# AdrianoEttari/DiffusionRemoteSensing

Measured on AMD Instinct MI355X. Metric: unet_denoise_steps_per_s, higher is better.
Workload: dtype f16 main + block-scaled fp6 (e2m3) cross terms of tap pairs on the wide 3x3 layers (FL, 11 of 11 launches of the dominant kernel); split bf16 x3 (hi + lo) everywhere else; f32 accumulate

## Files before the change

diffusionremotesensing_amd/csrc/attn_gate_sp.hip:

```cpp
#include "conv_epilogue.h"
#include "mfma_policy.h"

namespace {

template <int NT, bool PSI_ONLY = false>
__global__ __launch_bounds__(NT == 2 ? 1024 : 512, 1) void attn_gate_sp_kernel(AttnGateDesc d) {
  constexpr int THREADS = NT == 2 ? 1024 : 512, NW = THREADS / 64;
  extern __shared__ __attribute__((aligned(16))) char smem[];
  using P = PolicyBF16X3;
  constexpr int Ch = 16 * NT, NC = NT / 2;
  const int ncx = d.Cc / 32;
  const int gate_img = ncx * 4 * Ch * 16, wg_img = NC * 4 * Ch * 16, wx_img = NC * 16 * Ch * 16;
  char* sGate = smem;
  char* sWg = sGate + 2 * gate_img;
  char* sWx = sWg + 2 * wg_img;
  char* sRes = sWx + 2 * wx_img;
  float* sB = reinterpret_cast<float*>(sRes + 2 * wg_img);
  {
    const int tid = threadIdx.x;
    auto copy = [&](char* dst, const void* src, int bytes) {
      for (int o0 = tid * 16; o0 < bytes; o0 += 8 * THREADS * 16) {
        u32x4 v[8];
#pragma unroll
        for (int u = 0; u < 8; ++u) {
          const int o = o0 + u * THREADS * 16;
          if (o < bytes) v[u] = *reinterpret_cast<const u32x4*>(reinterpret_cast<const char*>(src) + o);
        }
#pragma unroll
        for (int u = 0; u < 8; ++u) {
          const int o = o0 + u * THREADS * 16;
          if (o < bytes) *reinterpret_cast<u32x4*>(dst + o) = v[u];
        }
      }
    };
    copy(sGate, d.w_gate, 2 * gate_img);
    copy(sWg, d.w_wg, 2 * wg_img);
    copy(sWx, d.w_wx, 2 * wx_img);
    if constexpr (!PSI_ONLY) copy(sRes, d.w_res, 2 * wg_img);
    for (int i = tid; i < Ch; i += THREADS) {
      sB[i] = d.b_gate[i];
      sB[Ch + i] = d.b_wg[i] + d.b_wx[i];
      sB[2 * Ch + i] = d.w_psi[i];
      sB[3 * Ch + i] = PSI_ONLY ? 0.f : d.b_res[i];
    }
    if (tid == 0) sB[4 * Ch] = d.b_psi[0];
  }
  __syncthreads();

  const int lane = threadIdx.x & 63, wave = threadIdx.x >> 6;
  const int lr = lane & 15, kg = lane >> 4;
  auto wfrag = [&](const char* base, int img, int slot) {
    return P::load(base, (size_t)img, (size_t)slot * 16);
  };
  const int bw = (d.LW + 15) / 16;
  const long long nitems = (long long)d.N * d.LH * bw;
  const int OW = 2 * d.LW, OH = 2 * d.LH;
  for (long long it = (long long)blockIdx.x * NW + wave; it < nitems; it += (long long)gridDim.x * NW) {
    const int xb = (int)(it % bw), y = (int)((it / bw) % d.LH), n = (int)(it / ((long long)bw * d.LH));
    const int px_raw = xb * 16 + lr;
    const bool valid = px_raw < d.LW;
    const int px = valid ? px_raw : d.LW - 1;
    typename P::Frag xr[4][NC];
#pragma unroll
    for (int t = 0; t < 4; ++t) {
      const size_t pix = ((size_t)n * OH + 2 * y + (t >> 1)) * OW + 2 * px + (t & 1);
      const char* g = reinterpret_cast<const char*>(d.xres) + (pix * d.r_cs + d.r_co) * 4 + kg * 16;
#pragma unroll
      for (int cc = 0; cc < NC; ++cc)
        xr[t][cc] = typename P::Frag{*reinterpret_cast<const bf16x8*>(g + cc * 128), *reinterpret_cast<const bf16x8*>(g + cc * 128 + 64)};
    }
    f32x4 acc[NT];
#pragma unroll
    for (int tt = 0; tt < NT; ++tt) acc[tt] = f32x4{0.f, 0.f, 0.f, 0.f};
    {
      const char* g = reinterpret_cast<const char*>(d.x) + ((((size_t)n * d.LH + y) * d.LW + px) * d.x_cs + d.x_co) * 4 + kg * 16;
      for (int c = 0; c < ncx; c += 2) {
        const typename P::Frag a0{*reinterpret_cast<const bf16x8*>(g + c * 128), *reinterpret_cast<const bf16x8*>(g + c * 128 + 64)};
        const typename P::Frag a1{*reinterpret_cast<const bf16x8*>(g + c * 128 + 128), *reinterpret_cast<const bf16x8*>(g + c * 128 + 192)};
#pragma unroll
        for (int tt = 0; tt < NT; ++tt) acc[tt] = P::mma(wfrag(sGate, gate_img, (c * 4 + kg) * Ch + tt * 16 + lr), a0, acc[tt]);
#pragma unroll
        for (int tt = 0; tt < NT; ++tt) acc[tt] = P::mma(wfrag(sGate, gate_img, ((c + 1) * 4 + kg) * Ch + tt * 16 + lr), a1, acc[tt]);
      }
    }
    typename P::Frag gfr[NC];
#pragma unroll
    for (int cc = 0; cc < NC; ++cc) {
      const float* bsrc = d.b_gate_img ? d.b_gate_img + (size_t)n * Ch + cc * 32 + kg * 8 : sB + cc * 32 + kg * 8;
      const float4 b0 = *reinterpret_cast<const float4*>(bsrc);
      const float4 b1 = *reinterpret_cast<const float4*>(bsrc + 4);
      const float bb[8] = {b0.x, b0.y, b0.z, b0.w, b1.x, b1.y, b1.z, b1.w};
      float v[8];
#pragma unroll
      for (int j = 0; j < 4; ++j) {
        v[j] = drs_maxf(acc[2 * cc][j] + bb[j], 0.f);
        v[4 + j] = drs_maxf(acc[2 * cc + 1][j] + bb[4 + j], 0.f);
      }
      u32x4 h, l;
      drs_sp_split8(v, h, l);
      gfr[cc] = typename P::Frag{__builtin_bit_cast(bf16x8, h), __builtin_bit_cast(bf16x8, l)};
    }
#pragma unroll
    for (int tt = 0; tt < NT; ++tt) acc[tt] = f32x4{0.f, 0.f, 0.f, 0.f};
#pragma unroll
    for (int cc = 0; cc < NC; ++cc)
#pragma unroll
      for (int tt = 0; tt < NT; ++tt) acc[tt] = P::mma(wfrag(sWg, wg_img, (cc * 4 + kg) * Ch + tt * 16 + lr), gfr[cc], acc[tt]);
    __builtin_amdgcn_sched_barrier(0);
#pragma unroll
    for (int t = 0; t < 4; ++t) {
#pragma unroll
      for (int cc = 0; cc < NC; ++cc)
#pragma unroll
        for (int tt = 0; tt < NT; ++tt)
          acc[tt] = P::mma(wfrag(sWx, wx_img, ((cc * 4 + t) * 4 + kg) * Ch + tt * 16 + lr), xr[t][cc], acc[tt]);
      __builtin_amdgcn_sched_barrier(0);
    }
    float dot = 0.f;
#pragma unroll
    for (int tt = 0; tt < NT; ++tt) {
      const int ch = (tt >> 1) * 32 + kg * 8 + (tt & 1) * 4;
      const float4 bs = *reinterpret_cast<const float4*>(sB + Ch + ch);
      const float4 wp = *reinterpret_cast<const float4*>(sB + 2 * Ch + ch);
      dot += drs_maxf(acc[tt][0] + bs.x, 0.f) * wp.x + drs_maxf(acc[tt][1] + bs.y, 0.f) * wp.y +
             drs_maxf(acc[tt][2] + bs.z, 0.f) * wp.z + drs_maxf(acc[tt][3] + bs.w, 0.f) * wp.w;
    }
    dot += __shfl_xor(dot, 16);
    dot += __shfl_xor(dot, 32);
    const float psi = 1.f / (1.f + expf(-(dot + sB[4 * Ch])));
    if (d.psi_out && valid && kg == 0) d.psi_out[((size_t)n * d.LH + y) * d.LW + px] = psi;
    if constexpr (!PSI_ONLY)
#pragma unroll
    for (int t = 0; t < 4; ++t) {
#pragma unroll
      for (int tt = 0; tt < NT; ++tt) acc[tt] = f32x4{0.f, 0.f, 0.f, 0.f};
#pragma unroll
      for (int cc = 0; cc < NC; ++cc)
#pragma unroll
        for (int tt = 0; tt < NT; ++tt) acc[tt] = P::mma(wfrag(sRes, wg_img, (cc * 4 + kg) * Ch + tt * 16 + lr), xr[t][cc], acc[tt]);
      __builtin_amdgcn_sched_barrier(0);
      const size_t pix = ((size_t)n * OH + 2 * y + (t >> 1)) * OW + 2 * px + (t & 1);
      char* o = reinterpret_cast<char*>(d.out) + (pix * d.out_cs + d.out_co) * 4 + kg * 16;
#pragma unroll
      for (int cc = 0; cc < NC; ++cc) {
        const float4 b0 = *reinterpret_cast<const float4*>(sB + 3 * Ch + cc * 32 + kg * 8);
        const float4 b1 = *reinterpret_cast<const float4*>(sB + 3 * Ch + cc * 32 + kg * 8 + 4);
        const float bb[8] = {b0.x, b0.y, b0.z, b0.w, b1.x, b1.y, b1.z, b1.w};
        float v[8];
#pragma unroll
        for (int j = 0; j < 4; ++j) {
          v[j] = psi * acc[2 * cc][j] + bb[j];
          v[4 + j] = psi * acc[2 * cc + 1][j] + bb[4 + j];
        }
        u32x4 h, l;
        drs_sp_split8(v, h, l);
        if (valid) {
          drs_store16(o + cc * 128, h);
          drs_store16(o + cc * 128 + 64, l);
        }
      }
    }
  }
}


template <int NCX>
__global__ __launch_bounds__(512, 1) void attn_gate_wide2_kernel(AttnGateDesc d) {
  using P = PolicyBF16X3;
  using Frag = typename P::Frag;
  constexpr int Ch = 128, NG = 4;
  constexpr int XB = 4 * NCX * 16 * 128;
  constexpr int TB = 4 * NG * 16 * 128;
  constexpr int RB = XB > 2 * TB ? XB : 2 * TB;
  extern __shared__ __attribute__((aligned(16))) char smem[];
  char* sX = smem;
  char* sG = smem + RB;
  float* sPsi = reinterpret_cast<float*>(sG + TB);
  float* sB = sPsi + 8 * 64;
  for (int i = threadIdx.x; i < Ch; i += 512) {
    sB[i] = d.b_wg[i] + d.b_wx[i];
    sB[Ch + i] = d.w_psi[i];
    sB[2 * Ch + i] = d.b_res[i];
  }
  if (threadIdx.x == 0) sB[3 * Ch] = d.b_psi[0];
  const int tid = threadIdx.x, lane = tid & 63, wave = __builtin_amdgcn_readfirstlane((int)(tid >> 6));
  const int lr = lane & 15, kg = lane >> 4;
  const int G = wave >> 1, th = wave & 1, ch0 = G * 32 + kg * 8 + th * 4;
  const size_t gate_img = (size_t)NCX * 4 * Ch * 16, wg_img = (size_t)NG * 4 * Ch * 16, wx_img = (size_t)NG * 16 * Ch * 16;
  const int bw = (d.LW + 15) / 16;
  const long long nblk16 = (long long)d.N * d.LH * bw;
  const long long nitems = (nblk16 + 3) / 4;
  const int OW = 2 * d.LW, OH = 2 * d.LH;
  typedef const __attribute__((address_space(1))) char* gptr;
  typedef const __attribute__((address_space(1))) bf16x8* gfrag;
  typedef const __attribute__((address_space(1))) u32x4* gquad;
  auto uni = [](const void* q) __attribute__((always_inline)) {
    gptr g = (gptr)q;
    asm volatile("" : "+s"(g));
    return g;
  };
  const gptr gw_gate = uni(d.w_gate), gw_wg = uni(d.w_wg), gw_wx = uni(d.w_wx), gw_res = uni(d.w_res);
  const gptr gx = uni(reinterpret_cast<const char*>(d.x) + (size_t)d.x_co * 4);
  const gptr gr = uni(reinterpret_cast<const char*>(d.xres) + (size_t)d.r_co * 4);
  const unsigned lane_w = (unsigned)((kg * Ch + wave * 16 + lr) * 16);
  auto opaque = [](unsigned v) __attribute__((always_inline)) { asm volatile("" : "+v"(v)); return v; };
  auto wfrag = [&](gptr base, size_t img, int urow) __attribute__((always_inline)) {
    const unsigned o = opaque(lane_w) + (unsigned)urow * (unsigned)(Ch * 16);
    return Frag{*(gfrag)(base + o), *(gfrag)(base + (o + (unsigned)img))};
  };
  auto afrag = [&](const char* img, int nc, int pb, int c) __attribute__((always_inline)) {
    const char* line = img + ((pb * nc + c) * 16 + lr) * 128;
    const int s0 = ((kg + lr) & 7) * 16;
    return Frag{*reinterpret_cast<const bf16x8*>(line + s0), *reinterpret_cast<const bf16x8*>(line + (s0 ^ 64))};
  };
  auto mfma = [](const bf16x8& w, const bf16x8& x, const f32x4& c) __attribute__((always_inline)) {
    return __builtin_amdgcn_mfma_f32_16x16x32_bf16(w, x, c, 0, 0, 0);
  };
  auto step4 = [&](const Frag& w, const Frag (&a)[4], f32x4 (&acc)[4]) __attribute__((always_inline)) {
#pragma unroll
    for (int b = 0; b < 4; ++b) acc[b] = mfma(w.lo, a[b].hi, acc[b]);
#pragma unroll
    for (int b = 0; b < 4; ++b) acc[b] = mfma(w.hi, a[b].lo, acc[b]);
#pragma unroll
    for (int b = 0; b < 4; ++b) acc[b] = mfma(w.hi, a[b].hi, acc[b]);
  };
  __syncthreads();
  for (long long it = blockIdx.x; it < nitems; it += gridDim.x) {
    unsigned xo[4], ro[4], oo[4];
    int nn[4], npx[4];
#pragma unroll
    for (int b = 0; b < 4; ++b) {
      const long long q = it * 4 + b;
      const long long qc = q < nblk16 ? q : nblk16 - 1;
      const int xb = (int)(qc % bw), y = (int)((qc / bw) % d.LH);
      nn[b] = (int)(qc / ((long long)bw * d.LH));
      npx[b] = q < nblk16 ? min(16, d.LW - xb * 16) : 0;
      xo[b] = (unsigned)((((size_t)nn[b] * d.LH + y) * d.LW + xb * 16) * d.x_cs * 4);
      ro[b] = (unsigned)((((size_t)nn[b] * OH + 2 * y) * OW + 2 * xb * 16) * d.r_cs * 4);
      oo[b] = (unsigned)((((size_t)nn[b] * OH + 2 * y) * OW + 2 * xb * 16) * d.out_cs * 4);
    }
    auto pick = [&](const unsigned (&v)[4], int b) __attribute__((always_inline)) { return b == 0 ? v[0] : b == 1 ? v[1] : b == 2 ? v[2] : v[3]; };
    auto picki = [&](const int (&v)[4], int b) __attribute__((always_inline)) { return b == 0 ? v[0] : b == 1 ? v[1] : b == 2 ? v[2] : v[3]; };
    u32x4 xr[8];
#pragma unroll
    for (int i = 0; i < 8; ++i) {
      const int e = i * 512 + tid, pix = e / (8 * NCX), pb = pix >> 4, pl = pix & 15;
      const int plc = min(pl, max(picki(npx, pb) - 1, 0));
      xr[i] = *(gquad)(gx + (pick(xo, pb) + (unsigned)(plc * d.x_cs * 4) + (unsigned)((e % (8 * NCX)) * 16)));
    }
    u32x4 tr[4];
    auto tap_load = [&](int t4) __attribute__((always_inline)) {
#pragma unroll
      for (int i = 0; i < 4; ++i) {
        const int e = i * 512 + tid, pix = e >> 5, pb = pix >> 4, pl = pix & 15;
        const int plc = min(pl, max(picki(npx, pb) - 1, 0));
        tr[i] = *(gquad)(gr + (pick(ro, pb) + (unsigned)((((t4 >> 1) * OW + 2 * plc + (t4 & 1)) * d.r_cs) * 4) + (unsigned)((e & 31) * 16)));
      }
    };
    auto tap_store = [&](int buf) __attribute__((always_inline)) {
#pragma unroll
      for (int i = 0; i < 4; ++i) {
        const int e = i * 512 + tid, pix = e >> 5, c = (e >> 3) & 3, sl = e & 7, pb = pix >> 4, pl = pix & 15;
        *reinterpret_cast<u32x4*>(sX + buf * TB + ((pb * NG + c) * 16 + pl) * 128 + ((sl + pl) & 7) * 16) = tr[i];
      }
    };
    tap_load(0);
    Frag wr[NG];
#pragma unroll
    for (int cc = 0; cc < NG; ++cc) wr[cc] = wfrag(gw_res, wg_img, cc * 4);
    constexpr int WD = 3, NST = NCX + NG + 4 * NG;
    Frag wq[WD + 1];
    auto wstep = [&](int st) __attribute__((always_inline)) {
      if (st < NCX) return wfrag(gw_gate, gate_img, st * 4);
      if (st < NCX + NG) return wfrag(gw_wg, wg_img, (st - NCX) * 4);
      const int t4 = (st - NCX - NG) / NG, cc = (st - NCX - NG) % NG;
      return wfrag(gw_wx, wx_img, (cc * 4 + t4) * 4);
    };
#pragma unroll
    for (int st = 0; st < WD; ++st) wq[st] = wstep(st);
#pragma unroll
    for (int i = 0; i < 8; ++i) {
      const int e = i * 512 + tid, pix = e / (8 * NCX), c = (e / 8) % NCX, sl = e & 7, pb = pix >> 4, pl = pix & 15;
      *reinterpret_cast<u32x4*>(sX + ((pb * NCX + c) * 16 + pl) * 128 + ((sl + pl) & 7) * 16) = xr[i];
    }
    __syncthreads();
    f32x4 acc[4];
#pragma unroll
    for (int b = 0; b < 4; ++b) acc[b] = f32x4{0.f, 0.f, 0.f, 0.f};
#pragma unroll
    for (int c = 0; c < NCX; ++c) {
      if (c + WD < NST) wq[(c + WD) % (WD + 1)] = wstep(c + WD);
      Frag a[4];
#pragma unroll
      for (int b = 0; b < 4; ++b) a[b] = afrag(sX, NCX, b, c);
      step4(wq[c % (WD + 1)], a, acc);
      __builtin_amdgcn_sched_barrier(0);
    }
    {
#pragma unroll
      for (int b = 0; b < 4; ++b) {
        const float* bsrc = (d.b_gate_img ? d.b_gate_img + (size_t)nn[b] * Ch : d.b_gate) + ch0;
        const float4 bb = *reinterpret_cast<const float4*>(bsrc);
        const float v[4] = {drs_maxf(acc[b][0] + bb.x, 0.f), drs_maxf(acc[b][1] + bb.y, 0.f), drs_maxf(acc[b][2] + bb.z, 0.f), drs_maxf(acc[b][3] + bb.w, 0.f)};
        unsigned h2[2], l2[2];
        drs_sp_split4(v, h2, l2);
        char* line = sG + ((b * NG + G) * 16 + lr) * 128;
        const int s0 = ((kg + lr) & 7) * 16 + th * 8;
        *reinterpret_cast<uint2*>(line + s0) = make_uint2(h2[0], h2[1]);
        *reinterpret_cast<uint2*>(line + (s0 ^ 64)) = make_uint2(l2[0], l2[1]);
      }
    }
    __syncthreads();
    tap_store(0);
    tap_load(1);
    __syncthreads();
#pragma unroll
    for (int b = 0; b < 4; ++b) acc[b] = f32x4{0.f, 0.f, 0.f, 0.f};
#pragma unroll
    for (int cc = 0; cc < NG; ++cc) {
      if (NCX + cc + WD < NST) wq[(NCX + cc + WD) % (WD + 1)] = wstep(NCX + cc + WD);
      Frag a[4];
#pragma unroll
      for (int b = 0; b < 4; ++b) a[b] = afrag(sG, NG, b, cc);
      step4(wq[(NCX + cc) % (WD + 1)], a, acc);
      __builtin_amdgcn_sched_barrier(0);
    }
    f32x4 att[4][4];
#pragma unroll
    for (int t4 = 0; t4 < 4; ++t4)
#pragma unroll
      for (int b = 0; b < 4; ++b) att[t4][b] = f32x4{0.f, 0.f, 0.f, 0.f};
#pragma unroll
    for (int t4 = 0; t4 < 4; ++t4) {
      if (t4 + 1 < 4) tap_store((t4 + 1) & 1);
      if (t4 + 2 < 4) tap_load(t4 + 2);
#pragma unroll
      for (int cc = 0; cc < NG; ++cc) {
        const int st = NCX + NG + t4 * NG + cc;
        if (st + WD < NST) wq[(st + WD) % (WD + 1)] = wstep(st + WD);
        Frag a[4];
#pragma unroll
        for (int b = 0; b < 4; ++b) a[b] = afrag(sX + (t4 & 1) * TB, NG, b, cc);
        step4(wq[st % (WD + 1)], a, acc);
        step4(wr[cc], a, att[t4]);
        __builtin_amdgcn_sched_barrier(0);
      }
      __syncthreads();
    }
    {
      const float4 bsum = *reinterpret_cast<const float4*>(sB + ch0), wp = *reinterpret_cast<const float4*>(sB + Ch + ch0);
#pragma unroll
      for (int b = 0; b < 4; ++b) {
        float dot = drs_maxf(acc[b][0] + bsum.x, 0.f) * wp.x + drs_maxf(acc[b][1] + bsum.y, 0.f) * wp.y +
                    drs_maxf(acc[b][2] + bsum.z, 0.f) * wp.z + drs_maxf(acc[b][3] + bsum.w, 0.f) * wp.w;
        dot += __shfl_xor(dot, 16);
        dot += __shfl_xor(dot, 32);
        if (kg == 0) sPsi[wave * 64 + b * 16 + lr] = dot;
      }
    }
    __syncthreads();
    {
      const float4 br = *reinterpret_cast<const float4*>(sB + 2 * Ch + ch0);
#pragma unroll
      for (int b = 0; b < 4; ++b) {
        const int i = b * 16 + lr;
        float sum = sB[3 * Ch];
#pragma unroll
        for (int w = 0; w < 8; ++w) sum += sPsi[w * 64 + i];
        const float psi = 1.f / (1.f + expf(-sum));
        const bool ok = lr < npx[b];
        if (d.psi_out && ok && kg == 0 && wave == 0) {
          const long long q = it * 4 + b;
          const int xb = (int)(q % bw), y = (int)((q / bw) % d.LH);
          d.psi_out[((size_t)nn[b] * d.LH + y) * d.LW + xb * 16 + lr] = psi;
        }
#pragma unroll
        for (int t4 = 0; t4 < 4; ++t4) {
          const float v[4] = {psi * att[t4][b][0] + br.x, psi * att[t4][b][1] + br.y, psi * att[t4][b][2] + br.z, psi * att[t4][b][3] + br.w};
          unsigned h2[2], l2[2];
          drs_sp_split4(v, h2, l2);
          if (ok) {
            char* o = reinterpret_cast<char*>(d.out) + (size_t)d.out_co * 4 + oo[b] +
                      (size_t)(((t4 >> 1) * OW + 2 * lr + (t4 & 1)) * d.out_cs + G * 32) * 4 + kg * 16 + th * 8;
            *reinterpret_cast<uint2*>(o) = make_uint2(h2[0], h2[1]);
            *reinterpret_cast<uint2*>(o + 64) = make_uint2(l2[0], l2[1]);
// ... 97 lines not shown
```

diffusionremotesensing_amd/csrc/conv_s2_sp.hip:

```cpp
#include <stdio.h>
#include <stdlib.h>

#include "conv_epilogue.h"
#include "mfma_policy.h"

namespace {

__device__ __forceinline__ void copy_weights(char* smem, const TapConv& d, int nck, int GC, int n0, unsigned w_gimage, int tid) {
  const int slots = nck * 36 * GC;
  const char* wsrc = reinterpret_cast<const char*>(d.w);
  for (int i0 = tid; i0 < 2 * slots; i0 += 512 * 8) {
    u32x4 v[8];
#pragma unroll
    for (int u = 0; u < 8; ++u) {
      const int i = i0 + u * 512;
      if (i < 2 * slots) {
        const int im = i >= slots, idx = im ? i - slots : i;
        const int r = idx / GC, j = idx - r * GC;
        v[u] = *reinterpret_cast<const u32x4*>(wsrc + (size_t)im * w_gimage + ((size_t)r * d.Cout + n0 + j) * 16);
      }
    }
#pragma unroll
    for (int u = 0; u < 8; ++u) {
      const int i = i0 + u * 512;
      if (i < 2 * slots) *reinterpret_cast<u32x4*>(smem + (size_t)i * 16) = v[u];
    }
  }
}

template <int NT>
__global__ __launch_bounds__(512, 1) void conv_s2_sp_kernel(TapConv d, int nck, unsigned w_gimage) {
  extern __shared__ __attribute__((aligned(16))) char smem[];
  using P = PolicyBF16X3;
  constexpr int GC = 16 * NT;
  const int tid = threadIdx.x, lane = tid & 63, wave = __builtin_amdgcn_readfirstlane(tid >> 6);
  const int lr = lane & 15, kg = lane >> 4;
  const int ngroups = d.Cout / GC;
  const int xcd = blockIdx.x & 7, j8 = blockIdx.x >> 3, nb8 = gridDim.x >> 3;
  const int grp = j8 % ngroups, member = j8 / ngroups, members = nb8 / ngroups;
  const int n0 = grp * GC;
  const int img = nck * 36 * GC * 16;
  copy_weights(smem, d, nck, GC, n0, w_gimage, tid);
  __syncthreads();

  const int bw = (d.OW + 15) / 16;
  const int rows = d.N * d.OH;
  const int r_lo = (int)((long long)rows * xcd / 8), r_hi = (int)((long long)rows * (xcd + 1) / 8);
  const int Q = (r_hi - r_lo) * bw;
  const int stride = members * 8, first = member * 8 + wave;
  const int my_items = first < Q ? (Q - first + stride - 1) / stride : 0;
  const int S = my_items * nck;
  if (S == 0) return;
  const int half = drs_sp_group_bytes(d.in_cs);
  const char* zero = reinterpret_cast<const char*>(d.zero_line) + kg * 16;
  const char* wbase = smem + ((size_t)kg * GC + lr) * 16;

  struct Taps { typename P::Frag c[3], r[3], e[3]; };
  Taps fa, fb;
  auto issue = [&](int s, Taps& f) __attribute__((always_inline)) {
    const int it = s / nck, c = s - it * nck;
    const int q = first + it * stride;
    const int row = r_lo + q / bw, xb = q - (q / bw) * bw;
    const int n = row / d.OH, y = row - n * d.OH;
    const int px = min(xb * 16 + lr, d.OW - 1);
    const int iy0 = 2 * y - 1, ix0 = 2 * px - 1;
    const char* base = reinterpret_cast<const char*>(d.in) +
                       ((((long long)n * d.H + iy0) * d.W + ix0) * d.in_cs + d.in_co) * 4 + c * 128 + kg * 16;
    const int rowb = d.W * d.in_cs * 4, pixb = d.in_cs * 4;
#pragma unroll
    for (int ky = 0; ky < 3; ++ky) {
      const bool row_ok = ky > 0 || iy0 >= 0;
      const char* pc = row_ok ? base + ky * rowb + pixb : zero;
      const char* pr = row_ok ? base + ky * rowb + 2 * pixb : zero;
      f.c[ky] = typename P::Frag{*reinterpret_cast<const bf16x8*>(pc), *reinterpret_cast<const bf16x8*>(row_ok ? pc + half : zero)};
      f.r[ky] = typename P::Frag{*reinterpret_cast<const bf16x8*>(pr), *reinterpret_cast<const bf16x8*>(row_ok ? pr + half : zero)};
      if (lr == 0) {
        const bool ok = row_ok && ix0 >= 0;
        const char* pe = ok ? base + ky * rowb : zero;
        f.e[ky] = typename P::Frag{*reinterpret_cast<const bf16x8*>(pe), *reinterpret_cast<const bf16x8*>(ok ? pe + half : zero)};
      }
    }
  };
  auto shift_in = [&](const bf16x8& edge, const bf16x8& right) __attribute__((always_inline)) {
    const u32x4 e = __builtin_bit_cast(u32x4, edge), r = __builtin_bit_cast(u32x4, right);
    u32x4 o;
#pragma unroll
    for (int j = 0; j < 4; ++j)
      o[j] = (unsigned)__builtin_amdgcn_update_dpp((int)e[j], (int)r[j], 0x111, 0xf, 0xf, false);
    return __builtin_bit_cast(bf16x8, o);
  };
  f32x4 acc[1][NT];
  float bias8[NT / 2][8];
#pragma unroll
  for (int pr = 0; pr < NT / 2; ++pr) {
    const float4 a = d.bias ? *reinterpret_cast<const float4*>(d.bias + n0 + pr * 32 + kg * 8) : make_float4(0.f, 0.f, 0.f, 0.f);
    const float4 b = d.bias ? *reinterpret_cast<const float4*>(d.bias + n0 + pr * 32 + kg * 8 + 4) : make_float4(0.f, 0.f, 0.f, 0.f);
    bias8[pr][0] = a.x; bias8[pr][1] = a.y; bias8[pr][2] = a.z; bias8[pr][3] = a.w;
    bias8[pr][4] = b.x; bias8[pr][5] = b.y; bias8[pr][6] = b.z; bias8[pr][7] = b.w;
  }
  auto store_row = [&](int n, int y, int x0) __attribute__((always_inline)) {
    const bool lo = lr < 8;
    const int pl = lr & 7;
#pragma unroll
    for (int pr = 0; pr < NT / 2; ++pr) {
      float v[8];
#pragma unroll
      for (int j = 0; j < 4; ++j) { v[j] = acc[0][2 * pr][j] + bias8[pr][j]; v[4 + j] = acc[0][2 * pr + 1][j] + bias8[pr][4 + j]; }
      if (d.relu_pre || d.relu_post) {
#pragma unroll
        for (int j = 0; j < 8; ++j) v[j] = drs_maxf(v[j], 0.f);
      }
      u32x4 H, L;
      drs_sp_split8(v, H, L);
      const u32x4 got = drs_dpp_swap8(lo ? L : H);
#pragma unroll
      for (int h = 0; h < 2; ++h) {
        const int tx = x0 + pl + 8 * h;
        if (tx < d.OW) {
          const size_t opix = ((size_t)n * d.OH + y) * d.OW + tx;
          char* gp = reinterpret_cast<char*>(d.out) + (opix * d.out_cs + d.out_co + n0 + pr * 32) * 4 + (lo ? 0 : 64) + kg * 16;
          drs_store16(gp, (h == 0) ? (lo ? H : got) : (lo ? got : L));
        }
      }
    }
  };
  auto compute = [&](int s, const Taps& f) __attribute__((always_inline)) {
    const int it = s / nck, c = s - it * nck;
    if (c == 0) {
#pragma unroll
      for (int t = 0; t < NT; ++t) acc[0][t] = f32x4{0.f, 0.f, 0.f, 0.f};
    }
    const char* wc = wbase + (size_t)c * 36 * GC * 16;
#pragma unroll
    for (int ky = 0; ky < 3; ++ky) {
      const typename P::Frag left{shift_in(f.e[ky].hi, f.r[ky].hi), shift_in(f.e[ky].lo, f.r[ky].lo)};
#pragma unroll
      for (int kx = 0; kx < 3; ++kx) {
        const typename P::Frag& a = kx == 0 ? left : (kx == 1 ? f.c[ky] : f.r[ky]);
#pragma unroll
        for (int t = 0; t < NT; ++t) {
          const typename P::Frag wf = P::load(wc, (size_t)img, (size_t)((ky * 3 + kx) * 4 * GC + t * 16) * 16);
          acc[0][t] = P::mma(wf, a, acc[0][t]);
        }
      }
      __builtin_amdgcn_sched_barrier(0);
    }
    if (c == nck - 1) {
      const int q = first + it * stride;
      const int row = r_lo + q / bw, xb = q - (q / bw) * bw;
      const int n = row / d.OH, y = row - n * d.OH;
      store_row(n, y, xb * 16);
    }
  };
  issue(0, fa);
  for (int s = 0; s < S; s += 2) {
    if (s + 1 < S) issue(s + 1, fb);
    compute(s, fa);
    if (s + 2 < S) issue(s + 2, fa);
    if (s + 1 < S) compute(s + 1, fb);
  }
}


template <int NT>
__global__ __launch_bounds__(512, 1) void convt_sp_kernel(TapConv d, int nck, unsigned w_gimage) {
  extern __shared__ __attribute__((aligned(16))) char smem[];
  using P = PolicyBF16X3;
  constexpr int GC = 16 * NT;
  const int tid = threadIdx.x, lane = tid & 63, wave = __builtin_amdgcn_readfirstlane(tid >> 6);
  const int lr = lane & 15, kg = lane >> 4;
  const int ngroups = d.Cout / GC;
  const int xcd = blockIdx.x & 7, j8 = blockIdx.x >> 3, nb8 = gridDim.x >> 3;
  const int grp = j8 % ngroups, member = j8 / ngroups, members = nb8 / ngroups;
  const int n0 = grp * GC;
  const int img = nck * 36 * GC * 16;
  copy_weights(smem, d, nck, GC, n0, w_gimage, tid);
  __syncthreads();

  const int bw = d.W / 16;
  const int rows = d.N * (d.H >> 1);
  const int r_lo = (int)((long long)rows * xcd / 8), r_hi = (int)((long long)rows * (xcd + 1) / 8);
  const int Q = (r_hi - r_lo) * bw;
  const int stride = members * 8, first = member * 8 + wave;
  const int my_items = first < Q ? (Q - first + stride - 1) / stride : 0;
  const int S = my_items * nck;
  if (S == 0) return;
  const int half = drs_sp_group_bytes(d.in_cs);
  const char* zero = reinterpret_cast<const char*>(d.zero_line) + kg * 16;
  const char* wbase = smem + ((size_t)kg * GC + lr) * 16;

  struct Rows { typename P::Frag a[3], e[3]; };
  Rows fa, fb;
  auto issue = [&](int s, Rows& f) __attribute__((always_inline)) {
    const int it = s / nck, c = s - it * nck;
    const int q = first + it * stride;
    const int row = r_lo + q / bw, xb = q - (q / bw) * bw;
    const int hh = d.H >> 1;
    const int n = row / hh, y = 2 * (row - n * hh);
    const int px = xb * 16 + lr;
    const char* base = reinterpret_cast<const char*>(d.in) +
                       ((((long long)n * d.H + y) * d.W + px) * d.in_cs + d.in_co) * 4 + c * 128 + kg * 16;
    const int rowb = d.W * d.in_cs * 4, pixb = d.in_cs * 4;
#pragma unroll
    for (int dy = 0; dy < 3; ++dy) {
      const bool row_ok = y + dy < d.H;
      const char* p = row_ok ? base + dy * rowb : zero;
      f.a[dy] = typename P::Frag{*reinterpret_cast<const bf16x8*>(p), *reinterpret_cast<const bf16x8*>(row_ok ? p + half : zero)};
      if (lr == 15) {
        const bool ok = row_ok && px + 1 < d.W;
        const char* pe = ok ? base + dy * rowb + pixb : zero;
        f.e[dy] = typename P::Frag{*reinterpret_cast<const bf16x8*>(pe), *reinterpret_cast<const bf16x8*>(ok ? pe + half : zero)};
      }
    }
  };
  auto shift_in = [&](const bf16x8& edge, const bf16x8& own) __attribute__((always_inline)) {
    const u32x4 e = __builtin_bit_cast(u32x4, edge), r = __builtin_bit_cast(u32x4, own);
    u32x4 o;
#pragma unroll
    for (int j = 0; j < 4; ++j)
      o[j] = (unsigned)__builtin_amdgcn_update_dpp((int)e[j], (int)r[j], 0x101, 0xf, 0xf, false);
    return __builtin_bit_cast(bf16x8, o);
  };
  f32x4 acc[2][4][NT];
  float bias8[NT / 2][8];
#pragma unroll
  for (int pr = 0; pr < NT / 2; ++pr) {
    const float4 a = d.bias ? *reinterpret_cast<const float4*>(d.bias + n0 + pr * 32 + kg * 8) : make_float4(0.f, 0.f, 0.f, 0.f);
    const float4 b = d.bias ? *reinterpret_cast<const float4*>(d.bias + n0 + pr * 32 + kg * 8 + 4) : make_float4(0.f, 0.f, 0.f, 0.f);
    bias8[pr][0] = a.x; bias8[pr][1] = a.y; bias8[pr][2] = a.z; bias8[pr][3] = a.w;
    bias8[pr][4] = b.x; bias8[pr][5] = b.y; bias8[pr][6] = b.z; bias8[pr][7] = b.w;
  }
  auto store_item = [&](int r, int n, int y, int x0) __attribute__((always_inline)) {
    const bool lo = lr < 8;
    const int pl = lr & 7;
#pragma unroll
    for (int ph = 0; ph < 4; ++ph)
#pragma unroll
      for (int pr = 0; pr < NT / 2; ++pr) {
        float v[8];
#pragma unroll
        for (int j = 0; j < 4; ++j) { v[j] = acc[r][ph][2 * pr][j] + bias8[pr][j]; v[4 + j] = acc[r][ph][2 * pr + 1][j] + bias8[pr][4 + j]; }
        u32x4 H, L;
        drs_sp_split8(v, H, L);
        const u32x4 got = drs_dpp_swap8(lo ? L : H);
        const size_t orow = ((size_t)n * d.OH + 2 * y + (ph >> 1)) * d.OW;
#pragma unroll
        for (int h = 0; h < 2; ++h) {
          const size_t opix = orow + 2 * (x0 + pl + 8 * h) + (ph & 1);
          char* gp = reinterpret_cast<char*>(d.out) + (opix * d.out_cs + d.out_co + n0 + pr * 32) * 4 + (lo ? 0 : 64) + kg * 16;
          drs_store16(gp, (h == 0) ? (lo ? H : got) : (lo ? got : L));
        }
      }
  };
  auto compute = [&](int s, const Rows& f) __attribute__((always_inline)) {
    const int it = s / nck, c = s - it * nck;
    if (c == 0) {
#pragma unroll
      for (int r = 0; r < 2; ++r)
#pragma unroll
        for (int ph = 0; ph < 4; ++ph)
#pragma unroll
          for (int t = 0; t < NT; ++t) acc[r][ph][t] = f32x4{0.f, 0.f, 0.f, 0.f};
    }
    const char* wc = wbase + (size_t)c * 36 * GC * 16;
    typename P::Frag right[3];
#pragma unroll
    for (int i = 0; i < 3; ++i) right[i] = typename P::Frag{shift_in(f.e[i].hi, f.a[i].hi), shift_in(f.e[i].lo, f.a[i].lo)};
#pragma unroll
    for (int dy = 0; dy < 2; ++dy) {
#pragma unroll
      for (int dx = 0; dx < 2; ++dx) {
#pragma unroll
        for (int ky = 0; ky < 3; ++ky)
#pragma unroll
          for (int kx = 0; kx < 3; ++kx) {
            if ((ky == 0 ? 1 : 0) != dy || (kx == 0 ? 1 : 0) != dx) continue;
            const int ph = (ky == 1 ? 0 : 1) * 2 + (kx == 1 ? 0 : 1);
#pragma unroll
            for (int t = 0; t < NT; ++t) {
              const typename P::Frag wf = P::load(wc, (size_t)img, (size_t)((ky * 3 + kx) * 4 * GC + t * 16) * 16);
#pragma unroll
              for (int r = 0; r < 2; ++r) acc[r][ph][t] = P::mma(wf, dx == 0 ? f.a[r + dy] : right[r + dy], acc[r][ph][t]);
            }
          }
        __builtin_amdgcn_sched_barrier(0);
      }
    }
    if (c == nck - 1) {
      const int q = first + it * stride;
      const int row = r_lo + q / bw, xb = q - (q / bw) * bw;
      const int hh = d.H >> 1;
      const int n = row / hh, y = 2 * (row - n * hh);
      store_item(0, n, y, xb * 16);
      store_item(1, n, y + 1, xb * 16);
    }
  };
  issue(0, fa);
  for (int s = 0; s < S; s += 2) {
    if (s + 1 < S) issue(s + 1, fb);
    compute(s, fa);
    if (s + 2 < S) issue(s + 2, fa);
    if (s + 1 < S) compute(s + 1, fb);
  }
}

template <int NT, bool CONVT = false>
int s2_launch(const TapConv& d, int nck, unsigned w_gimage, hipStream_t s) {
  auto kern = CONVT ? convt_sp_kernel<2> : conv_s2_sp_kernel<NT>;
  const size_t lds = (size_t)2 * nck * 36 * 16 * NT * 16;
  int num_cu = 0;
  {
    const int rc = drs_kernel_prepare(reinterpret_cast<const void*>(kern), 160 * 1024, &num_cu);
    if (rc) return rc;
  }
  const int ngroups = d.Cout / (16 * NT);
  int per_xcd = num_cu / 8;
  per_xcd = per_xcd / ngroups * ngroups;
  if (per_xcd < ngroups) per_xcd = ngroups;
  DRS_LAUNCH(kern, dim3((unsigned)(8 * per_xcd)), dim3(512), lds, s, d, nck, w_gimage);
  DRS_CHECK_HIP(hipGetLastError());
  return DRS_OK;
}

int s2_tiles(const TapConv& d) {
  const int nck = d.Cin / 32;
  const size_t budget = 156 * 1024;
  if (d.Cout % 64 == 0 && d.Cout <= 64 && (size_t)2 * nck * 36 * 64 * 16 <= budget) return 4;
  if ((size_t)2 * nck * 36 * 32 * 16 <= budget) return 2;
  return 0;
}

}

bool drs_conv_s2_sp_supported(const TapConv& d, int impl) {
  static const int env = getenv("DRS_S2K") ? atoi(getenv("DRS_S2K")) : 1;
  if (!env || impl != DRS_IMPL_MFMA_BF16X3) return false;
  if (!d.in || !d.in_sp || !d.out || !d.out_sp || !d.zero_line || d.mode != 0 || d.ntaps != 9 || d.wtaps_total != 9) return false;
  if (d.in_stride != 2 || d.out_scale != 1 || d.out_oy || d.out_ox) return false;
  for (int i = 0; i < 9; ++i)
    if (d.dy[i] != i / 3 - 1 || d.dx[i] != i % 3 - 1 || d.wtap[i] != i) return false;
  if (d.in2 || d.out2 || d.fuse_out || d.dual || d.gate || d.in_add || d.res || d.sigmoid || d.out_nchw) return false;
  if ((d.H & 1) || (d.W & 1) || d.OH != d.H / 2 || d.OW != d.W / 2 || d.TH != d.OH || d.TW != d.OW) return false;
  if (d.Cin % 32 || d.Cout % 32 || (d.in_cs & 31) || (d.in_co & 31) || (d.out_cs & 31) || (d.out_co & 31)) return false;
  if (d.post_add || d.bias2) return false;
  return s2_tiles(d) != 0;
}

int drs_launch_conv_s2_sp(const TapConv& d, hipStream_t s) {
  const int nck = d.Cin / 32;
  const unsigned w_gimage = (unsigned)((size_t)nck * 9 * 4 * d.Cout * 16);
  return s2_tiles(d) == 4 ? s2_launch<4>(d, nck, w_gimage, s) : s2_launch<2>(d, nck, w_gimage, s);
}

bool drs_convt_sp_supported(const TapConv& d, int impl) {
  static const int env = getenv("DRS_S2K") ? atoi(getenv("DRS_S2K")) : 1;
  if (!env || impl != DRS_IMPL_MFMA_BF16X3) return false;
  if (!d.in || !d.in_sp || !d.out || !d.out_sp || !d.zero_line || d.mode != DRS_TAPMODE_CONVT || d.ntaps != 9 || d.wtaps_total != 9) return false;
  if (d.in_stride != 1 || d.out_scale != 2 || d.out_oy || d.out_ox) return false;
  for (int i = 0; i < 9; ++i)
    if (d.wtap[i] != i) return false;
  if (d.in2 || d.out2 || d.fuse_out || d.dual || d.gate || d.in_add || d.res || d.sigmoid || d.out_nchw) return false;
  if (d.post_add || d.bias2 || d.relu_pre || d.relu_post) return false;
  if ((d.W & 15) || (d.H & 1) || d.OH != 2 * d.H || d.OW != 2 * d.W || d.TH != d.H || d.TW != d.W) return false;
  if (d.Cin % 32 || d.Cout % 32 || (d.in_cs & 31) || (d.in_co & 31) || (d.out_cs & 31) || (d.out_co & 31)) return false;
  return (size_t)2 * (d.Cin / 32) * 36 * 32 * 16 <= 156 * 1024;
}

int drs_launch_convt_sp(const TapConv& d, hipStream_t s) {
  const int nck = d.Cin / 32;
  const unsigned w_gimage = (unsigned)((size_t)nck * 9 * 4 * d.Cout * 16);
  return s2_launch<2, true>(d, nck, w_gimage, s);
}
```

diffusionremotesensing_amd/csrc/upfuse_proj_sp.hip:

```cpp
#include <stdio.h>
#include <stdlib.h>

#include "conv_epilogue.h"
#include "mfma_policy.h"

namespace {

constexpr int RBC = 8;
struct RowOpU { PolicyBF16X3::Frag c, e; };

__device__ __forceinline__ bf16x8 dpp_shift_u(const bf16x8& edge, const bf16x8& own, bool left) {
  const u32x4 e = __builtin_bit_cast(u32x4, edge), r = __builtin_bit_cast(u32x4, own);
  u32x4 o;
#pragma unroll
  for (int j = 0; j < 4; ++j)
    o[j] = left ? (unsigned)__builtin_amdgcn_update_dpp((int)e[j], (int)r[j], 0x111, 0xf, 0xf, false)
                : (unsigned)__builtin_amdgcn_update_dpp((int)e[j], (int)r[j], 0x101, 0xf, 0xf, false);
  return __builtin_bit_cast(bf16x8, o);
}
__host__ __device__ constexpr int up_tap_p(int j) { return j >= 3 ? 1 : 0; }
__host__ __device__ constexpr int up_tap_t(int j) { return j >= 3 ? j - 2 : j; }
__host__ __device__ constexpr bool up_pair(int p, int t, int kv, int kw) { return p + kv - kw == 2 * (t - 1); }

template <int NCK>
__global__ __launch_bounds__(256, 3) void upfuse_proj_sp_kernel(UpFuseDesc d) {
  extern __shared__ __attribute__((aligned(16))) char smem[];
  using P = PolicyBF16X3;
  using Frag = typename P::Frag;
  constexpr int NR = RBC + 2, PF = 2;
  const int tid = threadIdx.x, lane = tid & 63, wave = __builtin_amdgcn_readfirstlane(tid >> 6);
  const int lr = lane & 15, kg = lane >> 4;
  constexpr int IMG = NCK * 5 * 4 * 16 * 16;
  char* sW = smem;
  float* sB = reinterpret_cast<float*>(smem + 2 * IMG);
  {
    const char* w = reinterpret_cast<const char*>(d.w);
    for (int o = tid * 16; o < 2 * IMG; o += 256 * 16) *reinterpret_cast<u32x4*>(sW + o) = *reinterpret_cast<const u32x4*>(w + o);
    if (tid < 4) sB[tid] = d.bias[min(tid, 3) * 8];
  }
  __syncthreads();
  const int OH = 2 * d.LH, OW = 2 * d.LW;
  const int gx = (d.LW + 15) >> 4, gy = (d.LH + RBC - 1) / RBC;
  const int total = d.N * gy * gx;
  const int xcd = blockIdx.x & 7, member = blockIdx.x >> 3, members = gridDim.x >> 3;
  const int t_lo = (int)((long long)total * xcd / 8), t_hi = (int)((long long)total * (xcd + 1) / 8);
  const int stride = members * 4, first = member * 4 + wave;
  const int pixb = d.in_cs * 4;
  const char* zero = reinterpret_cast<const char*>(d.zero_line) + kg * 16;
  const char* wlane = sW + ((size_t)kg * 16 + lr) * 16;
  const size_t plane = (size_t)OH * OW;
  const float bk = sB[kg];
  const int ko = min(kg, d.fuse_dim - 1);
  for (int q0 = t_lo + first; q0 < t_hi; q0 += stride) {
    int q = q0;
    const int x0 = (q % gx) * 16; q /= gx;
    const int m0 = (q % gy) * RBC;
    const int n = q / gy;
    const int cx = x0 + lr;
    const bool own_ok = cx < d.LW && kg < d.fuse_dim;
    RowOpU R[PF + 1][NCK];
    auto load_row = [&](int slot, int wr) __attribute__((always_inline)) {
      const int iy = m0 - 1 + wr;
      const bool ok = iy >= 0 && iy < d.LH && cx < d.LW;
      const char* base = reinterpret_cast<const char*>(d.in) +
                         ((((long long)n * d.LH + iy) * d.LW + cx) * d.in_cs + d.in_co) * 4 + kg * 16;
#pragma unroll
      for (int c = 0; c < NCK; ++c) {
        const char* p = ok ? base + c * 128 : zero;
        R[slot][c].c = Frag{*reinterpret_cast<const bf16x8*>(p), *reinterpret_cast<const bf16x8*>(ok ? p + 64 : zero)};
      }
      if (lr == 0 || lr == 15) {
        const int ex = lr == 0 ? x0 - 1 : x0 + 16;
        const bool eok = iy >= 0 && iy < d.LH && ex >= 0 && ex < d.LW;
        const char* be = reinterpret_cast<const char*>(d.in) +
                         ((((long long)n * d.LH + iy) * d.LW + ex) * d.in_cs + d.in_co) * 4 + kg * 16;
#pragma unroll
        for (int c = 0; c < NCK; ++c) {
          const char* pe = eok ? be + c * 128 : zero;
          R[slot][c].e = Frag{*reinterpret_cast<const bf16x8*>(pe), *reinterpret_cast<const bf16x8*>(eok ? pe + 64 : zero)};
        }
      }
      (void)pixb;
    };
    float* obase = d.fuse_out + ((size_t)n * d.fuse_dim + ko) * plane + 2 * min(cx, d.LW - 1);
    f32x4 S[3][2];
#pragma unroll
    for (int i = 0; i < PF; ++i) load_row(i, i);
#pragma unroll
    for (int wr = 0; wr < NR; ++wr) {
      if (wr + PF < NR) load_row((wr + PF) % (PF + 1), wr + PF);
      __builtin_amdgcn_sched_barrier(0);
      f32x4 s0 = {0.f, 0.f, 0.f, 0.f}, s1 = {0.f, 0.f, 0.f, 0.f};
#pragma unroll
      for (int c = 0; c < NCK; ++c) {
        const RowOpU& r = R[wr % (PF + 1)][c];
#pragma unroll
        for (int tx = 0; tx < 3; ++tx) {
          const Frag a = tx == 1 ? r.c : Frag{dpp_shift_u(r.e.hi, r.c.hi, tx == 0), dpp_shift_u(r.e.lo, r.c.lo, tx == 0)};
          const int g0 = tx == 0 ? 0 : (tx == 1 ? 1 : 3);
          s0 = P::mma(P::load(wlane, (size_t)IMG, (size_t)((c * 5 + g0) * 4 * 16) * 16), a, s0);
          if (tx >= 1) s1 = P::mma(P::load(wlane, (size_t)IMG, (size_t)((c * 5 + g0 + 1) * 4 * 16) * 16), a, s1);
        }
      }
      S[wr % 3][0] = s0;
      S[wr % 3][1] = s1;
      __builtin_amdgcn_sched_barrier(0);
      if (wr >= 2) {
        const int m = m0 + wr - 2;
        const f32x4(&A)[2] = S[(wr - 2) % 3];
        const f32x4(&B)[2] = S[(wr - 1) % 3];
        const f32x4(&C)[2] = S[wr % 3];
        float v[2][2][3];
#pragma unroll
        for (int px = 0; px < 2; ++px)
#pragma unroll
          for (int o = 0; o < 3; ++o) {
            auto pick = [&](const f32x4& t, int row) __attribute__((always_inline)) { return __shfl(t[row & 3], lr + 16 * (row >> 2), 64); };
            v[0][px][o] = pick(A[px], 0 + o) + pick(B[px], 3 + o) + pick(C[px], 6 + o);
            v[1][px][o] = pick(B[px], 9 + o) + pick(C[px], 12 + o);
          }
        if (m < d.LH) {
#pragma unroll
          for (int py = 0; py < 2; ++py) {
            const int oy = 2 * m + py;
            float w0 = kg == 0 ? v[py][0][0] : (kg == 1 ? v[py][0][1] : v[py][0][2]);
            float w1 = kg == 0 ? v[py][1][0] : (kg == 1 ? v[py][1][1] : v[py][1][2]);
            float2* op = reinterpret_cast<float2*>(obase + (size_t)oy * OW);
            float2 prev = make_float2(0.f, 0.f);
            if (own_ok && d.fuse_acc) prev = *op;
            w0 += bk + prev.x;
            w1 += bk + prev.y;
            if (d.eh && own_ok) {
              const int ch = ko * 8;
              if (oy == 0 || oy == OH - 1) {
                const float* e = d.eh + (((size_t)n * 2 + (oy ? 1 : 0)) * OW + 2 * cx) * d.Ch + ch;
                w0 += e[0];
                w1 += e[d.Ch];
              } else {
                if (cx == 0) w0 += d.ev[(((size_t)n * 2 + 0) * OH + oy) * d.Ch + ch];
                if (2 * cx + 1 == OW - 1) w1 += d.ev[(((size_t)n * 2 + 1) * OH + oy) * d.Ch + ch];
              }
            }
            if (own_ok) *op = make_float2(w0, w1);
          }
        }
      }
    }
  }
}

__global__ __launch_bounds__(128) void upfuse_proj_pack_kernel(const float* __restrict__ vp, const float* __restrict__ t_w, int Cc,
                                                               int Ch, int fuse_dim, char* __restrict__ dst) {
  const int nck = Cc >> 5;
  const int nslots = nck * 5 * 4 * 16;
  const size_t img = (size_t)nslots * 16;
  const int cinv = Cc + Ch;
  for (int s = blockIdx.x * 128 + threadIdx.x; s < nslots; s += gridDim.x * 128) {
    const int row = s & 15, q = (s >> 4) & 3, g = (s >> 6) % 5, ck = s / 320;
    const int j = row / 3, o = row - 3 * j;
    float x[8] = {0.f, 0.f, 0.f, 0.f, 0.f, 0.f, 0.f, 0.f};
    if (row < 15 && o < fuse_dim) {
      const int tx = g == 0 ? 0 : (g <= 2 ? 1 : 2), px = (g == 2 || g == 4) ? 1 : 0, py = up_tap_p(j), ty = up_tap_t(j);
      const int ci0 = ck * 32 + q * 8;
      for (int kvy = 0; kvy < 3; ++kvy)
        for (int kwy = 0; kwy < 3; ++kwy) {
          if (!up_pair(py, ty, kvy, kwy)) continue;
          for (int kvx = 0; kvx < 3; ++kvx)
            for (int kwx = 0; kwx < 3; ++kwx) {
              if (!up_pair(px, tx, kvx, kwx)) continue;
              const float* vq = vp + (size_t)(8 * o) * cinv * 9 + kvy * 3 + kvx;
              const float* wq = t_w + (size_t)ci0 * Cc * 9 + kwy * 3 + kwx;
              for (int c = 0; c < Cc; ++c) {
                const float vv = vq[(size_t)c * 9];
#pragma unroll
                for (int e = 0; e < 8; ++e) x[e] += vv * wq[((size_t)e * Cc + c) * 9];
              }
            }
        }
    }
    PolicyBF16X3::cvt_store(dst, img, (size_t)s * 16, x);
  }
}

}

size_t drs_upfuse_proj_weight_bytes(int Cc) { return (size_t)2 * (Cc / 32) * 5 * 4 * 16 * 16; }

bool drs_upfuse_proj_supported(int Cc, int Ch, int fuse_dim) {
  return Ch == 32 && (Cc == 32 || Cc == 64) && fuse_dim >= 1 && fuse_dim <= 3;
}

int drs_launch_upfuse_proj_pack(const float* vp, const float* t_w, int Cc, int Ch, int fuse_dim, void* dst, hipStream_t s) {
  DRS_REQUIRE(vp && t_w && dst && drs_upfuse_proj_supported(Cc, Ch, fuse_dim), DRS_ERR_SHAPE, "upfuse_proj_pack: Cc=%d Ch=%d fuse_dim=%d", Cc, Ch, fuse_dim);
  const int nslots = (Cc / 32) * 5 * 4 * 16;
  DRS_LAUNCH(upfuse_proj_pack_kernel, dim3((nslots + 127) / 128), dim3(128), 0, s, vp, t_w, Cc, Ch, fuse_dim, (char*)dst);
  DRS_CHECK_HIP(hipGetLastError());
  return DRS_OK;
}

int drs_launch_upfuse_proj(const UpFuseDesc& d, hipStream_t s) {
  DRS_REQUIRE(d.in && d.w && d.bias && d.zero_line && d.fuse_out && d.proj && !d.res && !d.out && !d.out2, DRS_ERR_ARG, "upfuse_proj: bad descriptor");
  DRS_REQUIRE(drs_upfuse_proj_supported(d.Cc, d.Ch, d.fuse_dim) && (d.in_cs & 31) == 0 && (d.in_co & 31) == 0, DRS_ERR_SHAPE, "upfuse_proj: channels");
  DRS_REQUIRE((d.eh == nullptr) == (d.ev == nullptr), DRS_ERR_ARG, "upfuse_proj: edge vectors");
  if ((size_t)d.N * d.LH * d.LW == 0) return DRS_OK;
  int num_cu = 0;
  const void* kern = d.Cc == 64 ? reinterpret_cast<const void*>(upfuse_proj_sp_kernel<2>) : reinterpret_cast<const void*>(upfuse_proj_sp_kernel<1>);
  {
    const int rc = drs_kernel_prepare(kern, 0, &num_cu);
    if (rc) return rc;
  }
  const size_t lds = drs_upfuse_proj_weight_bytes(d.Cc) + 64;
  const long long strips = (long long)d.N * ((d.LH + RBC - 1) / RBC) * ((d.LW + 15) >> 4);
  long long blocks = (long long)num_cu * 3;
  if (blocks * 4 > strips) blocks = (strips + 3) / 4;
  blocks = (blocks + 7) / 8 * 8;
  if (d.Cc == 64) DRS_LAUNCH(upfuse_proj_sp_kernel<2>, dim3((unsigned)blocks), dim3(256), lds, s, d);
  else DRS_LAUNCH(upfuse_proj_sp_kernel<1>, dim3((unsigned)blocks), dim3(256), lds, s, d);
  DRS_CHECK_HIP(hipGetLastError());
  return DRS_OK;
}
```

Before: 837.9.

## Prefetch epilogue operands and overlap weight staging with first input loads

Gate bias loads in the attention-gate kernels are hoisted ahead of the main MMA loop so their latency hides behind compute. The stride-2 conv kernels now issue the first activation fetch before copying weights into LDS, and use a wider register batch for that copy. The upfuse projection kernel prefetches its epilogue inputs (previous output and edge vectors) together with row loads, deepens the row prefetch to 3, and drops occupancy from 3 to 2 blocks per CU. The cost is higher register pressure and lower occupancy in exchange for better latency hiding.

New measurement: 837.3, median of 2. No clear change (-0.1%).

```diff
diff --git a/diffusionremotesensing_amd/csrc/attn_gate_sp.hip b/diffusionremotesensing_amd/csrc/attn_gate_sp.hip
--- a/diffusionremotesensing_amd/csrc/attn_gate_sp.hip
+++ b/diffusionremotesensing_amd/csrc/attn_gate_sp.hip
@@ -69,6 +69,15 @@
       for (int cc = 0; cc < NC; ++cc)
         xr[t][cc] = typename P::Frag{*reinterpret_cast<const bf16x8*>(g + cc * 128), *reinterpret_cast<const bf16x8*>(g + cc * 128 + 64)};
     }
+    float4 gb[NC][2];
+    if (d.b_gate_img) {
+#pragma unroll
+      for (int cc = 0; cc < NC; ++cc) {
+        const float* bsrc = d.b_gate_img + (size_t)n * Ch + cc * 32 + kg * 8;
+        gb[cc][0] = *reinterpret_cast<const float4*>(bsrc);
+        gb[cc][1] = *reinterpret_cast<const float4*>(bsrc + 4);
+      }
+    }
     f32x4 acc[NT];
 #pragma unroll
     for (int tt = 0; tt < NT; ++tt) acc[tt] = f32x4{0.f, 0.f, 0.f, 0.f};
@@ -86,9 +95,9 @@
     typename P::Frag gfr[NC];
 #pragma unroll
     for (int cc = 0; cc < NC; ++cc) {
-      const float* bsrc = d.b_gate_img ? d.b_gate_img + (size_t)n * Ch + cc * 32 + kg * 8 : sB + cc * 32 + kg * 8;
-      const float4 b0 = *reinterpret_cast<const float4*>(bsrc);
-      const float4 b1 = *reinterpret_cast<const float4*>(bsrc + 4);
+      const float* bsrc = sB + cc * 32 + kg * 8;
+      const float4 b0 = d.b_gate_img ? gb[cc][0] : *reinterpret_cast<const float4*>(bsrc);
+      const float4 b1 = d.b_gate_img ? gb[cc][1] : *reinterpret_cast<const float4*>(bsrc + 4);
       const float bb[8] = {b0.x, b0.y, b0.z, b0.w, b1.x, b1.y, b1.z, b1.w};
       float v[8];
 #pragma unroll
@@ -248,6 +257,10 @@
       const int plc = min(pl, max(picki(npx, pb) - 1, 0));
       xr[i] = *(gquad)(gx + (pick(xo, pb) + (unsigned)(plc * d.x_cs * 4) + (unsigned)((e % (8 * NCX)) * 16)));
     }
+    float4 gb[4];
+#pragma unroll
+    for (int b = 0; b < 4; ++b)
+      gb[b] = *reinterpret_cast<const float4*>((d.b_gate_img ? d.b_gate_img + (size_t)nn[b] * Ch : d.b_gate) + ch0);
     u32x4 tr[4];
     auto tap_load = [&](int t4) __attribute__((always_inline)) {
 #pragma unroll
@@ -299,8 +312,7 @@
     {
 #pragma unroll
       for (int b = 0; b < 4; ++b) {
-        const float* bsrc = (d.b_gate_img ? d.b_gate_img + (size_t)nn[b] * Ch : d.b_gate) + ch0;
-        const float4 bb = *reinterpret_cast<const float4*>(bsrc);
+        const float4 bb = gb[b];
         const float v[4] = {drs_maxf(acc[b][0] + bb.x, 0.f), drs_maxf(acc[b][1] + bb.y, 0.f), drs_maxf(acc[b][2] + bb.z, 0.f), drs_maxf(acc[b][3] + bb.w, 0.f)};
         unsigned h2[2], l2[2];
         drs_sp_split4(v, h2, l2);
diff --git a/diffusionremotesensing_amd/csrc/conv_s2_sp.hip b/diffusionremotesensing_amd/csrc/conv_s2_sp.hip
--- a/diffusionremotesensing_amd/csrc/conv_s2_sp.hip
+++ b/diffusionremotesensing_amd/csrc/conv_s2_sp.hip
@@ -6,13 +6,14 @@
 
 namespace {
 
+constexpr int WCOPY = 20;
 __device__ __forceinline__ void copy_weights(char* smem, const TapConv& d, int nck, int GC, int n0, unsigned w_gimage, int tid) {
   const int slots = nck * 36 * GC;
   const char* wsrc = reinterpret_cast<const char*>(d.w);
-  for (int i0 = tid; i0 < 2 * slots; i0 += 512 * 8) {
-    u32x4 v[8];
-#pragma unroll
-    for (int u = 0; u < 8; ++u) {
+  for (int i0 = tid; i0 < 2 * slots; i0 += 512 * WCOPY) {
+    u32x4 v[WCOPY];
+#pragma unroll
+    for (int u = 0; u < WCOPY; ++u) {
       const int i = i0 + u * 512;
       if (i < 2 * slots) {
         const int im = i >= slots, idx = im ? i - slots : i;
@@ -21,7 +22,7 @@
       }
     }
 #pragma unroll
-    for (int u = 0; u < 8; ++u) {
+    for (int u = 0; u < WCOPY; ++u) {
       const int i = i0 + u * 512;
       if (i < 2 * slots) *reinterpret_cast<u32x4*>(smem + (size_t)i * 16) = v[u];
     }
@@ -40,8 +41,6 @@
   const int grp = j8 % ngroups, member = j8 / ngroups, members = nb8 / ngroups;
   const int n0 = grp * GC;
   const int img = nck * 36 * GC * 16;
-  copy_weights(smem, d, nck, GC, n0, w_gimage, tid);
-  __syncthreads();
 
   const int bw = (d.OW + 15) / 16;
   const int rows = d.N * d.OH;
@@ -50,7 +49,6 @@
   const int stride = members * 8, first = member * 8 + wave;
   const int my_items = first < Q ? (Q - first + stride - 1) / stride : 0;
   const int S = my_items * nck;
-  if (S == 0) return;
   const int half = drs_sp_group_bytes(d.in_cs);
   const char* zero = reinterpret_cast<const char*>(d.zero_line) + kg * 16;
   const char* wbase = smem + ((size_t)kg * GC + lr) * 16;
@@ -152,7 +150,10 @@
       store_row(n, y, xb * 16);
     }
   };
-  issue(0, fa);
+  if (S > 0) issue(0, fa);
+  __builtin_amdgcn_sched_barrier(0);
+  copy_weights(smem, d, nck, GC, n0, w_gimage, tid);
+  __syncthreads();
   for (int s = 0; s < S; s += 2) {
     if (s + 1 < S) issue(s + 1, fb);
     compute(s, fa);
@@ -174,8 +175,6 @@
   const int grp = j8 % ngroups, member = j8 / ngroups, members = nb8 / ngroups;
   const int n0 = grp * GC;
   const int img = nck * 36 * GC * 16;
-  copy_weights(smem, d, nck, GC, n0, w_gimage, tid);
-  __syncthreads();
 
   const int bw = d.W / 16;
   const int rows = d.N * (d.H >> 1);
@@ -184,7 +183,6 @@
   const int stride = members * 8, first = member * 8 + wave;
   const int my_items = first < Q ? (Q - first + stride - 1) / stride : 0;
   const int S = my_items * nck;
-  if (S == 0) return;
   const int half = drs_sp_group_bytes(d.in_cs);
   const char* zero = reinterpret_cast<const char*>(d.zero_line) + kg * 16;
   const char* wbase = smem + ((size_t)kg * GC + lr) * 16;
@@ -295,7 +293,10 @@
       store_item(1, n, y + 1, xb * 16);
     }
   };
-  issue(0, fa);
+  if (S > 0) issue(0, fa);
+  __builtin_amdgcn_sched_barrier(0);
+  copy_weights(smem, d, nck, GC, n0, w_gimage, tid);
+  __syncthreads();
   for (int s = 0; s < S; s += 2) {
     if (s + 1 < S) issue(s + 1, fb);
     compute(s, fa);
diff --git a/diffusionremotesensing_amd/csrc/upfuse_proj_sp.hip b/diffusionremotesensing_amd/csrc/upfuse_proj_sp.hip
--- a/diffusionremotesensing_amd/csrc/upfuse_proj_sp.hip
+++ b/diffusionremotesensing_amd/csrc/upfuse_proj_sp.hip
@@ -23,11 +23,11 @@
 __host__ __device__ constexpr bool up_pair(int p, int t, int kv, int kw) { return p + kv - kw == 2 * (t - 1); }
 
 template <int NCK>
-__global__ __launch_bounds__(256, 3) void upfuse_proj_sp_kernel(UpFuseDesc d) {
+__global__ __launch_bounds__(256, 2) void upfuse_proj_sp_kernel(UpFuseDesc d) {
   extern __shared__ __attribute__((aligned(16))) char smem[];
   using P = PolicyBF16X3;
   using Frag = typename P::Frag;
-  constexpr int NR = RBC + 2, PF = 2;
+  constexpr int NR = RBC + 2, PF = 3;
   const int tid = threadIdx.x, lane = tid & 63, wave = __builtin_amdgcn_readfirstlane(tid >> 6);
   const int lr = lane & 15, kg = lane >> 4;
   constexpr int IMG = NCK * 5 * 4 * 16 * 16;
@@ -59,6 +59,30 @@
     const int cx = x0 + lr;
     const bool own_ok = cx < d.LW && kg < d.fuse_dim;
     RowOpU R[PF + 1][NCK];
+    float* obase = d.fuse_out + ((size_t)n * d.fuse_dim + ko) * plane + 2 * min(cx, d.LW - 1);
+    struct EpiIn { float2 prev[2]; float e0[2], e1[2]; };
+    EpiIn E[PF + 1];
+    auto edge_class = [&](int oy) __attribute__((always_inline)) { return oy == 0 || oy == OH - 1; };
+    auto load_epi = [&](int slot, int wr) __attribute__((always_inline)) {
+      const int m = m0 + wr - 2;
+      if (wr < 2 || m >= d.LH || !own_ok) return;
+#pragma unroll
+      for (int py = 0; py < 2; ++py) {
+        const int oy = 2 * m + py;
+        if (d.fuse_acc) E[slot].prev[py] = *reinterpret_cast<const float2*>(obase + (size_t)oy * OW);
+        if (d.eh) {
+          const int ch = ko * 8;
+          if (edge_class(oy)) {
+            const float* e = d.eh + (((size_t)n * 2 + (oy ? 1 : 0)) * OW + 2 * cx) * d.Ch + ch;
+            E[slot].e0[py] = e[0];
+            E[slot].e1[py] = e[d.Ch];
+          } else {
+            if (cx == 0) E[slot].e0[py] = d.ev[(((size_t)n * 2 + 0) * OH + oy) * d.Ch + ch];
+            if (2 * cx + 1 == OW - 1) E[slot].e1[py] = d.ev[(((size_t)n * 2 + 1) * OH + oy) * d.Ch + ch];
+          }
+        }
+      }
+    };
     auto load_row = [&](int slot, int wr) __attribute__((always_inline)) {
       const int iy = m0 - 1 + wr;
       const bool ok = iy >= 0 && iy < d.LH && cx < d.LW;
@@ -81,8 +105,8 @@
         }
       }
       (void)pixb;
+      load_epi(slot, wr);
     };
-    float* obase = d.fuse_out + ((size_t)n * d.fuse_dim + ko) * plane + 2 * min(cx, d.LW - 1);
     f32x4 S[3][2];
 #pragma unroll
     for (int i = 0; i < PF; ++i) load_row(i, i);
@@ -126,19 +150,18 @@
             float w0 = kg == 0 ? v[py][0][0] : (kg == 1 ? v[py][0][1] : v[py][0][2]);
             float w1 = kg == 0 ? v[py][1][0] : (kg == 1 ? v[py][1][1] : v[py][1][2]);
             float2* op = reinterpret_cast<float2*>(obase + (size_t)oy * OW);
+            const EpiIn& ei = E[wr % (PF + 1)];
             float2 prev = make_float2(0.f, 0.f);
-            if (own_ok && d.fuse_acc) prev = *op;
+            if (own_ok && d.fuse_acc) prev = ei.prev[py];
             w0 += bk + prev.x;
             w1 += bk + prev.y;
             if (d.eh && own_ok) {
-              const int ch = ko * 8;
-              if (oy == 0 || oy == OH - 1) {
-                const float* e = d.eh + (((size_t)n * 2 + (oy ? 1 : 0)) * OW + 2 * cx) * d.Ch + ch;
-                w0 += e[0];
-                w1 += e[d.Ch];
+              if (edge_class(oy)) {
+                w0 += ei.e0[py];
+                w1 += ei.e1[py];
               } else {
-                if (cx == 0) w0 += d.ev[(((size_t)n * 2 + 0) * OH + oy) * d.Ch + ch];
-                if (2 * cx + 1 == OW - 1) w1 += d.ev[(((size_t)n * 2 + 1) * OH + oy) * d.Ch + ch];
+                if (cx == 0) w0 += ei.e0[py];
+                if (2 * cx + 1 == OW - 1) w1 += ei.e1[py];
               }
             }
             if (own_ok) *op = make_float2(w0, w1);
@@ -211,7 +234,7 @@
   }
   const size_t lds = drs_upfuse_proj_weight_bytes(d.Cc) + 64;
   const long long strips = (long long)d.N * ((d.LH + RBC - 1) / RBC) * ((d.LW + 15) >> 4);
-  long long blocks = (long long)num_cu * 3;
+  long long blocks = (long long)num_cu * 2;
   if (blocks * 4 > strips) blocks = (strips + 3) / 4;
   blocks = (blocks + 7) / 8 * 8;
   if (d.Cc == 64) DRS_LAUNCH(upfuse_proj_sp_kernel<2>, dim3((unsigned)blocks), dim3(256), lds, s, d);
```
